# turswiming/UnSAMFlow

Measured on AMD Instinct MI355X. Metric: image-pairs/sec PWCLite fwd+bwd, KITTI 832x256 d=4, higher is better.
Workload: dtype f32; 1 GPU; PWCLite fwd(with_bk)+unFlowLoss+bwd+Adam, KITTI 832x256, d=4; global_batch=8, per_gpu_batch=8, max_displacement=4, parallelism=dp1

## Files before the change

### unsamflow_amd/_lib.py

```python
from __future__ import annotations

import ctypes
import os
import threading
from pathlib import Path

import torch

_LIB_PATH = Path(os.environ.get("USF_LIB", Path(__file__).resolve().parent / "lib" / "libunsamflow_hip.so"))
ABI_VERSION = 8
PAD_ZEROS = 0
PAD_BORDER = 1

_c_float_p = ctypes.c_void_p
_SIGNATURES = {
    "usf_abi_version": ([], ctypes.c_int),
    "usf_last_error_string": ([], ctypes.c_char_p),
    "usf_build_id": ([], ctypes.c_char_p),
    "usf_corr_fwd_f32": (
        [_c_float_p, _c_float_p, _c_float_p] + [ctypes.c_int] * 5 + [ctypes.c_void_p],
        ctypes.c_int,
    ),
    "usf_corr_bwd_f32": (
        [_c_float_p] * 5 + [ctypes.c_int] * 5 + [ctypes.c_void_p],
# ... 153 lines not shown
        [_c_float_p] * 3 + [ctypes.c_longlong] + [_c_float_p] * 8 + [ctypes.c_int] * 3 + [ctypes.c_void_p],
        ctypes.c_int,
    ),
    "usf_ar_loss_partials": ([ctypes.c_int] * 3, ctypes.c_int),
    "usf_ar_loss_fwd_f32": (
        [_c_float_p] + _ar_strided + [_c_float_p] * 3 + [ctypes.c_int] * 3 + [ctypes.c_float] * 2 + [ctypes.c_void_p],
        ctypes.c_int,
    ),
    "usf_ar_loss_bwd_f32": (
        [_c_float_p] + _ar_strided + [_c_float_p] * 3 + [ctypes.c_int] * 3 + [ctypes.c_float] * 2 + [ctypes.c_void_p],
        ctypes.c_int,
    ),
}

SEGPOOL_API_VERSION = 1
SEGPOOL_MAX_K = 1024
DEVERR_SEGPOOL_BAD_ID = 4
SEGPOOL_SYMBOLS = {
    "usf_segpool_api_version": ([], ctypes.c_int),
    "usf_segpool_state_words": ([ctypes.c_int] * 3, ctypes.c_longlong),
    "usf_segpool_fwd_f32": (
        [_c_float_p] * 3 + [ctypes.c_void_p] + [ctypes.c_int] * 5 + [ctypes.c_void_p],
        ctypes.c_int,
    ),
    "usf_segpool_bwd_f32": (
        [_c_float_p] * 2 + [ctypes.c_void_p] + [_c_float_p] * 2 + [ctypes.c_int] * 5 + [ctypes.c_void_p],
        ctypes.c_int,
    ),
}

HG_API_VERSION = 1
HG_MAX_K = 1024
HG_SLOTS = 6
HG_RECORD_WORDS = 16
HG_DEFAULT_HYP = 256
HG_STATUS = ("accepted", "too few reliable", "low reliable share", "low inlier share", "degenerate", "empty slot")
DEVERR_HG_BAD_ID = 8
_hg_flow = [_c_float_p, ctypes.c_longlong, _c_float_p]
HG_SYMBOLS = {
    "usf_hg_api_version": ([], ctypes.c_int),
    "usf_hg_workspace_bytes": ([ctypes.c_int] * 5, ctypes.c_longlong),
    "usf_hg_fit_f32": (
        _hg_flow + [_c_float_p, ctypes.c_int, ctypes.c_float, ctypes.c_int, ctypes.c_ulonglong, ctypes.c_void_p,
                    ctypes.c_void_p, ctypes.c_longlong] + [ctypes.c_int] * 3 + [ctypes.c_void_p],
        ctypes.c_int,
    ),
    "usf_hg_loss_partials": ([ctypes.c_int] * 3, ctypes.c_int),
    "usf_hg_loss_fwd_f32": (
        _hg_flow + [ctypes.c_void_p, ctypes.c_void_p, _c_float_p] + [ctypes.c_int] * 3 + [ctypes.c_void_p],
        ctypes.c_int,
    ),
    "usf_hg_loss_bwd_f32": (
        _hg_flow + [ctypes.c_void_p, _c_float_p, _c_float_p] + [ctypes.c_int] * 3 + [ctypes.c_void_p],
        ctypes.c_int,
    ),
}

_lock = threading.Lock()
_lib = None
_load_error: str | None = None


def library_path() -> Path:
    return _LIB_PATH


def load() -> ctypes.CDLL:
    global _lib, _load_error
    if _lib is not None:
        return _lib
    with _lock:
        if _lib is not None:
            return _lib
        if not _LIB_PATH.exists():
            _load_error = (
                f"libunsamflow_hip.so not found at {_LIB_PATH}; build it with "
                "`python -m unsamflow_amd.build` (hipcc, gfx950)"
            )
            raise RuntimeError(_load_error)
        lib = ctypes.CDLL(str(_LIB_PATH), mode=ctypes.RTLD_LOCAL)
        for name, (argtypes, restype) in {**_SIGNATURES, **CENSUS_SYMBOLS, **AR_SYMBOLS, **SEGPOOL_SYMBOLS,
                                          **HG_SYMBOLS}.items():
            fn = getattr(lib, name)
            fn.argtypes = argtypes
            fn.restype = restype
        v = lib.usf_abi_version()
        if v != ABI_VERSION:
            raise RuntimeError(f"libunsamflow_hip.so ABI version {v} != expected {ABI_VERSION}")
        v = lib.usf_census_api_version()
        if v != CENSUS_API_VERSION:
            raise RuntimeError(f"libunsamflow_hip.so census API version {v} != expected {CENSUS_API_VERSION}")
        v = lib.usf_ar_api_version()
        if v != AR_API_VERSION:
            raise RuntimeError(f"libunsamflow_hip.so AR API version {v} != expected {AR_API_VERSION}")
        v = lib.usf_segpool_api_version()
        if v != SEGPOOL_API_VERSION:
            raise RuntimeError(f"libunsamflow_hip.so segpool API version {v} != expected {SEGPOOL_API_VERSION}")
        v = lib.usf_hg_api_version()
        if v != HG_API_VERSION:
            raise RuntimeError(f"libunsamflow_hip.so hg API version {v} != expected {HG_API_VERSION}")
        _lib = lib
        return lib


def build_id() -> str:
    return load().usf_build_id().decode()


def is_available() -> bool:
    try:
        load()
        return True
    except (RuntimeError, OSError):
        return False


def check(rc: int, what: str) -> None:
    if rc != 0:
        msg = load().usf_last_error_string()
        msg = msg.decode() if msg else ""
        raise RuntimeError(f"{what} failed (rc={rc}): {msg}")


def stream_handle(device: torch.device) -> int:
    return torch.cuda.current_stream(device).cuda_stream
```

### unsamflow_amd/build.py

```python
from __future__ import annotations

import argparse
import hashlib
import os
import subprocess
import sys
from pathlib import Path

PKG_DIR = Path(__file__).resolve().parent
CSRC = PKG_DIR / "csrc"
LIB_DIR = PKG_DIR / "lib"
LIB_PATH = LIB_DIR / "libunsamflow_hip.so"
INCLUDE_DIR = PKG_DIR.parent / "include"

ARCH = os.environ.get("USF_OFFLOAD_ARCH", "gfx950")
HIPCC = os.environ.get("HIPCC", "/opt/rocm/bin/hipcc")

SOURCES = ["corr.hip", "warp.hip", "occ.hip", "photo.hip", "census.hip", "ar.hip", "segpool.hip", "hg.hip", "upsample.hip", "convex.hip", "stream.hip", "capi.cpp"]
HEADERS = ["usf_common.h", "warp_tap.h", "interp_tap.h", "strip.h", "wave.h", "scatter_rows.h", "seg_key.h"]
PUBLIC_HEADERS = ["unsamflow_hip.h", "unsamflow_hip_census.h", "unsamflow_hip_ar.h", "unsamflow_hip_segpool.h",
                  "unsamflow_hip_hg.h"]

COMMON_FLAGS = [
    "-O3",
    "-std=c++17",
    "-fno-slp-vectorize",
    "-fPIC",
    f"--offload-arch={ARCH}",
    "-Wall",
    "-Wno-unused-function",
    f"-I{INCLUDE_DIR}",
]


def build_id() -> str:
    h = hashlib.sha256()
    for f in [CSRC / s for s in SOURCES] + [CSRC / s for s in HEADERS] + [INCLUDE_DIR / s for s in PUBLIC_HEADERS]:
        h.update(f.name.encode())
        h.update(f.read_bytes())
    h.update(" ".join(COMMON_FLAGS).encode())
    return h.hexdigest()[:16]


def _stale(target: Path, deps: list[Path]) -> bool:
    if not target.exists():
        return True
    t = target.stat().st_mtime
    return any(d.stat().st_mtime > t for d in deps)


def build_library(force: bool = False, verbose: bool = False) -> Path:
    LIB_DIR.mkdir(exist_ok=True)
    obj_dir = LIB_DIR / "obj"
    obj_dir.mkdir(exist_ok=True)
    headers = [CSRC / h for h in HEADERS] + [INCLUDE_DIR / h for h in PUBLIC_HEADERS]
    bid = build_id()
    stamp = obj_dir / "build_id.txt"
    id_changed = not stamp.exists() or stamp.read_text().strip() != bid
    objs = []
    for src in SOURCES:
        s = CSRC / src
        o = obj_dir / (s.stem + ".o")
        objs.append(o)
        if force or _stale(o, [s] + headers) or (src == "capi.cpp" and id_changed):
            lang = ["-x", "hip"] if src.endswith(".hip") else []
            extra = [f'-DUSF_BUILD_ID="{bid}"'] if src == "capi.cpp" else []
            cmd = [HIPCC, *COMMON_FLAGS, *extra, *lang, "-c", str(s), "-o", str(o)]
            _run(cmd, verbose)
    stamp.write_text(bid + "\n")
    if force or _stale(LIB_PATH, objs):
        tmp = LIB_PATH.with_suffix(".so.tmp")
        cmd = [HIPCC, f"--offload-arch={ARCH}", "-shared", "-fPIC", *map(str, objs), "-o", str(tmp)]
        _run(cmd, verbose)
        os.replace(tmp, LIB_PATH)
# ... 26 lines not shown
```

### unsamflow_amd/csrc/capi.cpp

```cpp
#include <hip/hip_runtime.h>

#include <climits>
#include <cstdint>
#include <cstdarg>
#include <cstdio>
#include <cstdlib>

#include "../../include/unsamflow_hip.h"
#include "../../include/unsamflow_hip_ar.h"
#include "../../include/unsamflow_hip_census.h"
#include "../../include/unsamflow_hip_hg.h"
#include "../../include/unsamflow_hip_segpool.h"
#include "usf_common.h"

namespace usf {

static thread_local char g_err[512] = "";

void set_error(const char* fmt, ...) {
  va_list ap;
  va_start(ap, fmt);
  vsnprintf(g_err, sizeof(g_err), fmt, ap);
  va_end(ap);
}

void clear_error() { g_err[0] = '\0'; }

static bool check_dims(const char* fn, int B, int C, int H, int W) {
  if (B <= 0 || C <= 0 || H <= 0 || W <= 0) {
    set_error("%s: non-positive shape B=%d C=%d H=%d W=%d", fn, B, C, H, W);
    return false;
  }
  const long long per_sample = (long long)C * H * W;
  const long long max_elems = 0x7FFFFFF0LL / 4 - 1;
  if (per_sample > max_elems || (long long)H * W * 81 > max_elems) {
    set_error("%s: per-sample tensor too large (C*H*W=%lld)", fn, per_sample);
    return false;
  }
  return true;
}

static bool sync_check() {
  static const bool on = [] {
    const char* v = getenv("USF_SYNC_CHECK");
    return v && v[0] == '1';
  }();
  return on;
}

static bool capturing(hipStream_t s) {
  hipStreamCaptureStatus st = hipStreamCaptureStatusNone;
  return hipStreamIsCapturing(s, &st) == hipSuccess && st != hipStreamCaptureStatusNone;
}

static bool sync_check_on(hipStream_t s) { return sync_check() && !capturing(s); }

static int pre_check(const char* fn, hipStream_t s) {
  if (!sync_check_on(s)) return 0;
  const hipError_t e = hipStreamSynchronize(s);
  if (e != hipSuccess) {
    fprintf(stderr, "[usf] %s: stream already faulted BEFORE this launch: %s\n", fn, hipGetErrorString(e));
    set_error("%s: stream faulted before launch: %s (%d)", fn, hipGetErrorString(e), (int)e);
    return (int)e;
// ... 1086 lines not shown
    }
  if (const int pe = pre_check(fn, (hipStream_t)stream)) return pe;
  return finish(fn, convex_pyr_fwd_launch(nlevel, flow, mask, out, H, W, B, factor, mask_scale, (hipStream_t)stream),
                (hipStream_t)stream);
}

int usf_convex_upsample_pyramid_bwd_f32(int nlevel, const float* const* flow, const float* const* mask,
                                        const float* const* grad_out, float* const* grad_flow,
                                        float* const* grad_mask, float* scratch, long long scratch_floats,
                                        const int* H, const int* W, int B, int factor, float mask_scale,
                                        void* stream) {
  clear_error();
  const char* fn = "usf_convex_upsample_pyramid_bwd_f32";
  if (!check_convex_pyr(fn, nlevel, H, W, B, factor)) return USF_EINVAL;
  if (!flow || !mask || !grad_out) {
    set_error("%s: null input pointer array", fn);
    return USF_EINVAL;
  }
  for (int l = 0; l < nlevel; ++l)
    if (!flow[l] || !mask[l] || !grad_out[l] || (grad_flow && !grad_flow[l]) || (grad_mask && !grad_mask[l])) {
      set_error("%s: level %d: null pointer", fn, l);
      return USF_EINVAL;
    }
  if (grad_flow && (!scratch || scratch_floats < usf_convex_upsample_pyramid_bwd_scratch(nlevel, H, W, B))) {
    set_error("%s: grad_flow needs scratch of usf_convex_upsample_pyramid_bwd_scratch floats", fn);
    return USF_EINVAL;
  }
  if (!grad_flow && !grad_mask) return 0;
  if (const int pe = pre_check(fn, (hipStream_t)stream)) return pe;
  return finish(fn,
                convex_pyr_bwd_launch(nlevel, flow, mask, grad_out, grad_flow, grad_mask, scratch, H, W, B, factor,
                                      mask_scale, (hipStream_t)stream),
                (hipStream_t)stream);
}

int usf_area_pyramid_f32(const float* x, float* out1, float* out2, float* out3, int B, int C, int H,
                         int W, void* stream) {
  clear_error();
  const char* fn = "usf_area_pyramid_f32";
  if (!check_dims(fn, B, C, H, W)) return USF_EINVAL;
  if (H % 8 != 0 || W % 8 != 0) {
    set_error("%s: H=%d and W=%d must be multiples of 8", fn, H, W);
    return USF_EINVAL;
  }
  if (!x || !out1 || !out2 || !out3) {
    set_error("%s: null pointer", fn);
    return USF_EINVAL;
  }
  if (const int pe = pre_check(fn, (hipStream_t)stream)) return pe;
  return finish(fn, area_pyramid_launch(x, out1, out2, out3, (long long)B * C, H, W, (hipStream_t)stream),
                (hipStream_t)stream);
}

int usf_stream_copy_f32(const float* src, float* dst, long long n, void* stream) {
  clear_error();
  if (!src || !dst || n <= 0 || n % 4 != 0 || (reinterpret_cast<uintptr_t>(src) & 15) ||
      (reinterpret_cast<uintptr_t>(dst) & 15)) {
    set_error("usf_stream_copy_f32: need 16-byte aligned pointers and n %% 4 == 0 (n=%lld)", n);
    return USF_EINVAL;
  }
  if (const int pe = pre_check("usf_stream_copy_f32", (hipStream_t)stream)) return pe;
  return finish("usf_stream_copy_f32", stream_copy_launch(src, dst, n, (hipStream_t)stream), (hipStream_t)stream);
}

int usf_device_errors(void* stream, int clear) {
  clear_error();
  const int v = device_errors((hipStream_t)stream, clear != 0);
  if (v < 0) set_error("usf_device_errors: stream sync or flag read failed");
  return v;
}

int usf_set_variant(int op, int index) {
  clear_error();
  if (op < 0 || op > 3 || index < -1 || index >= variant_count(op)) {
    set_error("usf_set_variant: bad op %d / index %d", op, index);
    return USF_EINVAL;
  }
  set_variant_override(op, index);
  return variant_count(op);
}

}
```

### unsamflow_amd/csrc/usf_common.h

```cpp
#pragma once
#include <hip/hip_runtime.h>
#include <cstddef>
#include <cstdint>

#include "unsamflow_hip.h"

namespace usf {

int device_errors(hipStream_t s, bool clear, int mask = ~0);
template <class Sym>
int read_clear_flags(const Sym& word, bool clear, int mask = ~0) {
  int v = 0;
  if (hipMemcpyFromSymbol(&v, word, sizeof(int)) != hipSuccess) return -1;
  if (clear && (v & mask) != 0) {
    const int z = v & ~mask;
    if (hipMemcpyToSymbol(word, &z, sizeof(int)) != hipSuccess) return -1;
  }
  return v & mask;
}

void set_error(const char* fmt, ...);
void clear_error();

__host__ __device__ constexpr int round_up(int n, int m) { return ((n + m - 1) / m) * m; }
// ... 85 lines not shown
                                 int W, int pad_mode, float w_l1, float w_ssim, hipStream_t s);
hipError_t photo_pyr_fwd_launch(int nscale, const float* const* im1, const float* const* im2,
                                const float* const* mask1, const float* const* mask2, const float* const* flow,
                                const long long* fbs, const int* H, const int* W, float* partials, float* out,
                                float* const* basis, int B, int C, int pad_mode, float w_l1, float w_ssim,
                                hipStream_t s);
hipError_t photo_pyr_bwd_launch(int nscale, const float* const* basis, const float* coef, const float* gloss,
                                float* const* gflow, const int* H, const int* W, int B, int ndir, hipStream_t s);

int census_partials(int B, int H, int W);
hipError_t census_fwd_launch(const float* src, const float* tgt, const float* mask, const float* flow,
                             long long flow_bstride, float* partials, float* out, float* basis, int B, int H,
                             int W, int pad_mode, float w_ternary, hipStream_t s);
hipError_t census_pair_fwd_launch(const float* im1, const float* im2, const float* mask1, const float* mask2,
                                  const float* flow, long long flow_bstride, float* partials, float* out,
                                  float* basis, int B, int H, int W, int pad_mode, float w_ternary, hipStream_t s);
hipError_t census_pyr_fwd_launch(int nscale, const float* const* im1, const float* const* im2,
                                 const float* const* mask1, const float* const* mask2, const float* const* flow,
                                 const long long* fbs, const int* H, const int* W, float* partials, float* out,
                                 float* const* basis, int B, int pad_mode, float w_ternary, hipStream_t s);
hipError_t census_pyr_bwd_launch(int nscale, const float* const* basis, const float* coef, const float* gloss,
                                 float* const* gflow, const int* H, const int* W, int B, int ndir, hipStream_t s);

hipError_t ar_transform_launch(const float* img1, const float* img2, const float* flow, long long flow_bstride,
                               const float* mask, const float* theta, const float* noise1, const float* noise2,
                               float* img1_t, float* img2_t, float* flow_t, float* mask_t, int B, int H, int W,
                               hipStream_t s);
int ar_loss_partials(int B, int H, int W);
hipError_t ar_loss_fwd_launch(const float* pred, const float* target, long long tbs, long long tcs, long long trs,
                              const float* noc, long long nbs, long long nrs, const float* denom, float* partials,
                              float* out, int B, int H, int W, float eps, float q, hipStream_t s);
hipError_t ar_loss_bwd_launch(const float* pred, const float* target, long long tbs, long long tcs, long long trs,
                              const float* noc, long long nbs, long long nrs, const float* coef, const float* gloss,
                              float* gpred, int B, int H, int W, float eps, float q, hipStream_t s);

int segpool_device_errors(bool clear);
long long segpool_state_words(int B, int C, int K);
hipError_t segpool_fwd_launch(const float* proj, const float* seg, float* spread, unsigned* state, int B, int C,
                              int H, int W, int K, hipStream_t s);
hipError_t segpool_bwd_launch(const float* proj, const float* seg, const unsigned* state, const float* gs, float* gp,
                              int B, int C, int H, int W, int K, hipStream_t s);

int hg_device_errors(bool clear);
long long hg_workspace_bytes(int B, int H, int W, int K, int n_hyp);
hipError_t hg_fit_launch(const float* flow, long long fbs, const float* seg, const float* occ, int K, float thr,
                         int n_hyp, unsigned long long seed, int* records, void* workspace, int B, int H, int W,
                         hipStream_t s);
int hg_loss_partials(int B, int H, int W);
hipError_t hg_loss_fwd_launch(const float* flow, long long fbs, const float* seg, const int* records, double* partials,
                              float* out, int B, int H, int W, hipStream_t s);
hipError_t hg_loss_bwd_launch(const float* flow, long long fbs, const float* seg, const int* records,
                              const float* gloss, float* gflow, int B, int H, int W, hipStream_t s);

hipError_t upsample_fwd_launch(const float* x, float* out, int B, int C, int H, int W, int k,
                               hipStream_t s);
hipError_t upsample_bwd_launch(const float* gout, float* gx, int B, int C, int H, int W, int k,
                               hipStream_t s, const float* gout2 = nullptr);
int convex_pyramid_max_levels();
hipError_t convex_pyr_fwd_launch(int n, const float* const* flow, const float* const* mask, float* const* out,
                                 const int* H, const int* W, int B, int factor, float mask_scale, hipStream_t s);
hipError_t convex_pyr_bwd_launch(int n, const float* const* flow, const float* const* mask,
                                 const float* const* gout, float* const* gflow, float* const* gmask, float* scratch,
                                 const int* H, const int* W, int B, int factor, float mask_scale, hipStream_t s);
bool convex_factor_ok(int factor);
long long convex_bwd_scratch(int B, int H, int W);
hipError_t convex_fwd_launch(const float* flow, const float* mask, float* out, int B, int H, int W,
                             int factor, float mask_scale, hipStream_t s);
hipError_t convex_bwd_launch(const float* flow, const float* mask, const float* gout, float* gflow,
                             float* gmask, float* scratch, int B, int H, int W, int factor,
                             float mask_scale, hipStream_t s);
hipError_t stream_copy_launch(const float* src, float* dst, long long n, hipStream_t s);
hipError_t area_pyramid_launch(const float* x, float* o1, float* o2, float* o3, long long planes,
                               int H, int W, hipStream_t s);

}
```

### unsamflow_amd/kernel_timer.py

```python
from __future__ import annotations

import collections
import contextlib
import ctypes
import os

import torch

_active: "KernelTimer | None" = None
_roctx = None


def site_name(op: str, key) -> str:
    return "usf:" + op + ":" + "x".join(str(k) for k in key[:4]) + "".join(f":{k}" for k in key[4:])


def _roctx_lib():
    global _roctx
    if _roctx is None:
        _roctx = False
        if os.environ.get("USF_ROCTX") == "1":
            for name in ("librocprofiler-sdk-roctx.so.1", "librocprofiler-sdk-roctx.so", "libroctx64.so"):
                try:
                    lib = ctypes.CDLL(name)
# ... 57 lines not shown
        for a in agg.values():
            a["mean_us"] = a["total_us"] / a["n"]
        return agg


@contextlib.contextmanager
def timed(op: str, key, device, nbytes: int, flops: int = 0):
    rx = _roctx_lib()
    if rx:
        rx.roctxRangePushA(site_name(op, key).encode())
    try:
        kt = _active
        if kt is None or (kt.only is not None and (op, tuple(key)) not in kt.only):
            yield
            return
        if not kt.time_in_step:
            yield
            kt.records.append((op, key, None, None, nbytes, flops))
            return
        s = torch.cuda.Event(enable_timing=True)
        e = torch.cuda.Event(enable_timing=True)
        stream = torch.cuda.current_stream(device)
        s.record(stream)
        yield
        e.record(stream)
        kt.records.append((op, key, s, e, nbytes, flops))
    finally:
        if rx:
            rx.roctxRangePop()


def site_launcher(op: str, key, device, seed: int = 0):
    from . import ops

    g = torch.Generator(device=device).manual_seed(seed)
    if op == "corr_bwd_leaky":
        B, C, H, W = key[:4]
        x1 = torch.randn(B, C, H, W, device=device, generator=g)
        x2 = torch.randn(B, C, H, W, device=device, generator=g)
        cat = torch.randn(B, 81 + C + 2, H, W, device=device, generator=g)
        act = torch.nn.functional.leaky_relu(torch.randn(B, 81 + C + 2, H, W, device=device, generator=g), 0.1)
        mask = ops.corr_act_mask(B, H, W, 4, device, C=C)
        if mask is not None:
            ops.corr_forward_ex(x1, x2, 4, act[:, :81], 0.1, act_mask=mask)
        return lambda: ops.corr_backward_ex(x1, x2, cat[:, :81], 4, key[4], key[5], act_out=act[:, :81],
                                            act_mask=mask)
    if op == "corr_fwd_leaky":
        B, C, H, W = key[:4]
        x1 = torch.randn(B, C, H, W, device=device, generator=g)
        x2 = torch.randn(B, C, H, W, device=device, generator=g)
        cat = torch.empty(B, 81 + C + 2, H, W, device=device)
        mask = ops.corr_act_mask(B, H, W, 4, device, C=C)
        return lambda: ops.corr_forward_ex(x1, x2, 4, cat[:, :81], 0.1, act_mask=mask)
    if op in ("corr_fwd", "corr_bwd"):
        B, C, H, W = key[:4]
        x1 = torch.randn(B, C, H, W, device=device, generator=g)
        x2 = torch.randn(B, C, H, W, device=device, generator=g)
        if op == "corr_fwd":
            return lambda: ops.corr_forward(x1, x2, 4)
        need1, need2 = key[4], key[5]
        go = torch.randn(B, 81, H, W, device=device, generator=g)
        return lambda: ops.corr_backward(x1, x2, go, 4, need1, need2)
    if op in ("upsample", "upsample_bwd"):
        B, C, H, W, k = key[:5]
        if op == "upsample":
            f = torch.randn(B, C, H, W, device=device, generator=g)
            return lambda: ops.flow_upsample(f, k)
        go = torch.randn(B, C, H * k, W * k, device=device, generator=g)
        return lambda: ops.flow_upsample_backward(go, k)
    if op in ("convex_pyr", "convex_pyr_bwd"):
        B, f = key[0], key[-1]
        hw = [(key[i], key[i + 1]) for i in range(1, len(key) - 1, 2)]
        flows = [torch.randn(B, 2, h, w, device=device, generator=g) for h, w in hw]
        masks = [torch.randn(B, 9 * f * f, h, w, device=device, generator=g) for h, w in hw]
        if op == "convex_pyr":
            return lambda: ops.convex_upsample_pyramid(flows, masks, f)
        gos = [torch.randn(B, 2, f * h, f * w, device=device, generator=g) for h, w in hw]
        return lambda: ops.convex_upsample_pyramid_backward(flows, masks, gos, f)
    if op in ("convex_up", "convex_up_bwd"):
        B, H, W, f = key
        flow = torch.randn(B, 2, H, W, device=device, generator=g)
        mask = torch.randn(B, 9 * f * f, H, W, device=device, generator=g)
        if op == "convex_up":
            return lambda: ops.convex_upsample(flow, mask, f)
        go = torch.randn(B, 2, f * H, f * W, device=device, generator=g)
        return lambda: ops.convex_upsample_backward(flow, mask, go, f)
    if op == "area_pyramid":
        img = torch.rand(*key, device=device, generator=g)
        return lambda: ops.area_pyramid(img)
    if op == "photo_bwd":
        B, ndir, H, W = key
        basis = torch.randn(B, 4 * ndir, H, W, device=device, generator=g)
        coef = torch.rand(3 * ndir, device=device, generator=g)
        gl = torch.ones(ndir, device=device)
        return lambda: ops.photo_loss_backward(basis, coef, gl)
    if op == "census_bwd":
        B, ndir, H, W = key
        basis = torch.randn(B, 2 * ndir, H, W, device=device, generator=g)
        coef = torch.rand(2 * ndir, device=device, generator=g)
        gl = torch.ones(ndir, device=device)
        return lambda: ops.census_loss_backward(basis, coef, gl)
    if op in ("photo_pyr", "photo_pyr_grad", "photo_pyr_bwd", "census_pyr", "census_pyr_grad", "census_pyr_bwd"):
        B, C = key[:2]
        hw = [(key[i], key[i + 1]) for i in range(2, len(key) - (not op.endswith("_bwd")), 2)]
        if op == "census_pyr_bwd":
            bases = [torch.randn(B, 4, h, w, device=device, generator=g) for h, w in hw]
# ... 128 lines not shown
```

### unsamflow_amd/ops.py

```python
from __future__ import annotations

import ctypes
import weakref

import torch

from collections import OrderedDict, namedtuple

from . import _lib
from . import kernel_timer as _kt

PAD_MODES = {"zeros": _lib.PAD_ZEROS, "border": _lib.PAD_BORDER}


def _ptr(t: torch.Tensor | None) -> int | None:
    return None if t is None else t.data_ptr()


def _require_device_f32(name: str, t: torch.Tensor) -> None:
    if not isinstance(t, torch.Tensor):
        raise TypeError(f"{name} must be a torch.Tensor, got {type(t).__name__}")
    if t.device.type != "cuda":
        raise RuntimeError(
            f"unsamflow_amd: {name} is on {t.device}; the HIP kernels need tensors on a ROCm "
# ... 1000 lines not shown
    _args = (n, ptrs(fl), ptrs(mk), ptrs(outs), Hs, Ws, B, f_, float(mask_scale), _lib.stream_handle(dev),)
    with torch.cuda.device(dev), _kt.timed("convex_pyr", key, dev, nbytes):
        rc = lib.usf_convex_upsample_pyramid_f32(*_args)
    _lib.check(rc, "usf_convex_upsample_pyramid_f32")
    return outs


def convex_upsample_pyramid_backward(flows, masks, grad_outs, factor: int = 4, mask_scale: float = 0.25,
                                     need_flow: bool = True, need_mask: bool = True):
    import ctypes

    n = len(flows)
    fl = [f.contiguous() for f in flows]
    mk = [m.contiguous() for m in masks]
    go = [g.contiguous() for g in grad_outs]
    B, f_ = fl[0].shape[0], int(factor)
    if not (need_flow or need_mask):
        return None, None
    dev = fl[0].device
    gfs = [torch.empty((B, 2) + tuple(f.shape[2:]), device=dev, dtype=torch.float32) for f in fl] if need_flow else None
    gms = [torch.empty_like(m) for m in mk] if need_mask else None
    Hs, Ws = _level_sizes(fl)
    lib = _lib.load()
    nscr = int(lib.usf_convex_upsample_pyramid_bwd_scratch(n, Hs, Ws, B)) if need_flow else 0
    scratch = torch.empty(max(nscr, 1), device=dev, dtype=torch.float32)
    ptrs = lambda ts: _host_array(ctypes.c_void_p, [t.data_ptr() for t in ts])
    key = (B,) + tuple(v for f in fl for v in f.shape[2:]) + (f_,)
    ff = f_ * f_
    nbytes = sum(4 * B * f.shape[2] * f.shape[3] * (2 + 9 * ff + 2 * ff + (2 if need_flow else 0)
                                                    + (9 * ff if need_mask else 0)) for f in fl)
    _args = (n, ptrs(fl), ptrs(mk), ptrs(go), ptrs(gfs) if need_flow else None, ptrs(gms) if need_mask else None,
             scratch.data_ptr(), nscr, Hs, Ws, B, f_, float(mask_scale), _lib.stream_handle(dev),)
    with torch.cuda.device(dev), _kt.timed("convex_pyr_bwd", key, dev, nbytes):
        rc = lib.usf_convex_upsample_pyramid_bwd_f32(*_args)
    _lib.check(rc, "usf_convex_upsample_pyramid_bwd_f32")
    return gfs, gms


def area_pyramid(x: torch.Tensor):
    _require_device_f32("x", x)
    B, C, H, W = _nchw("x", x)
    if H % 8 or W % 8:
        raise ValueError(f"area_pyramid needs H, W multiples of 8, got {H}x{W}")
    xc = x.contiguous()
    outs = [torch.empty((B, C, H >> s, W >> s), device=x.device, dtype=torch.float32) for s in (1, 2, 3)]
    lib = _lib.load()
    nbytes = 4 * B * C * H * W * (1 + 1 / 4 + 1 / 16 + 1 / 64)
    _args = (xc.data_ptr(), outs[0].data_ptr(), outs[1].data_ptr(), outs[2].data_ptr(), B, C, H, W,
             _lib.stream_handle(x.device),)
    with torch.cuda.device(x.device), _kt.timed("area_pyramid", (B, C, H, W), x.device, int(nbytes)):
        rc = lib.usf_area_pyramid_f32(*_args)
    _lib.check(rc, "usf_area_pyramid_f32")
    return outs
```

### unsamflow_amd/pwclite.py

```python
from __future__ import annotations

from typing import Callable

import torch
import torch.nn as nn
import torch.nn.functional as F


def conv_block(cin: int, cout: int, k: int = 3, stride: int = 1, dilation: int = 1, relu: bool = True) -> nn.Sequential:
    layers = [nn.Conv2d(cin, cout, k, stride=stride, dilation=dilation, padding=((k - 1) * dilation) // 2, bias=True)]
    if relu:
        layers.append(nn.LeakyReLU(0.1, inplace=True))
    return nn.Sequential(*layers)


def full_segs_to_adj_maps(full_segs: torch.Tensor, win_size: int = 9, pad_mode: str = "replicate") -> torch.Tensor:
    r = (win_size - 1) // 2
    b, _, h, w = full_segs.shape
    nb = F.unfold(F.pad(full_segs, (r, r, r, r), mode=pad_mode), [win_size, win_size])
    return (full_segs == nb.reshape(b, win_size * win_size, h, w)).float()


class FeatureExtractor(nn.Module):
    def __init__(self, num_chs, input_adj_map: bool = False):
        super().__init__()
        self.num_chs = num_chs
        self.adj_map_net = None
        if input_adj_map:
            self.adj_map_net = nn.Sequential(
                conv_block(81, 32, k=1), conv_block(32, 32, stride=2), conv_block(32, 32),
                conv_block(32, 32, stride=2), conv_block(32, 32),
            )
        self.convs = nn.ModuleList()
        for lvl in range(len(num_chs) - 1):
            cin = num_chs[lvl] + (32 if input_adj_map and lvl == 2 else 0)
            cout = num_chs[lvl + 1]
            self.convs.append(nn.Sequential(conv_block(cin, cout, stride=2), conv_block(cout, cout)))

    def forward(self, x, adj_map=None):
        adj = self.adj_map_net(adj_map) if self.adj_map_net is not None else None
        pyramid = [x]
        for lvl, block in enumerate(self.convs):
            if adj is not None and lvl == 2:
                x = torch.cat((x, adj), dim=1)
            x = block(x)
            pyramid.append(x)
        return pyramid[::-1]


class FlowEstimatorDense(nn.Module):
    def __init__(self, ch_in: int):
        super().__init__()
        widths = [128, 128, 96, 64, 32]
        acc = ch_in
        for i, w in enumerate(widths, 1):
            setattr(self, f"conv{i}", conv_block(acc, w))
            acc += w
        self.feat_dim = acc
        self.conv_last = conv_block(acc, 2, relu=False)

    def forward(self, x):
        for i in range(1, 6):
            x = torch.cat([getattr(self, f"conv{i}")(x), x], dim=1)
        return x, self.conv_last(x)


# ... 15 lines not shown
        c = self.conv3(torch.cat([a, b], 1))
        d = self.conv4(torch.cat([b, c], 1))
        e = self.conv5(torch.cat([c, d], 1))
        return e, self.predict_flow(torch.cat([d, e], 1))


class ContextNetwork(nn.Module):
    def __init__(self, ch_in: int):
        super().__init__()
        self.convs = nn.Sequential(*[conv_block(ci, co, 3, 1, dil) for ci, co, dil in
                                     ((ch_in, 128, 1), (128, 128, 2), (128, 128, 4), (128, 96, 8))])
        self.flow_head = nn.Sequential(conv_block(96, 64, 3, 1, 16), conv_block(64, 32, 3, 1, 1),
                                       conv_block(32, 2, relu=False))

    def forward(self, x):
        feat = self.convs(x)
        return self.flow_head(feat), feat


class UpFlowNetwork(nn.Module):

    def __init__(self, ch_in: int = 96, scale_factor: int = 4):
        super().__init__()
        self.scale = scale_factor
        self.fused = False
        self.convs = nn.Sequential(conv_block(ch_in, 128, 3, 1, 1), conv_block(128, scale_factor ** 2 * 9, 3, 1, 1))

    def upsample_flow(self, flow, mask):
        N, _, H, W = flow.shape
        s = self.scale
        weights = torch.softmax(mask.view(N, 1, 9, s, s, H, W), dim=2)
        patches = F.unfold(s * flow, [3, 3], padding=1).view(N, 2, 9, 1, 1, H, W)
        up = torch.sum(weights * patches, dim=2)
        return up.permute(0, 1, 4, 2, 5, 3).reshape(N, 2, s * H, s * W)

    def mask(self, feat):
        return self.convs(feat)

    def forward(self, flow, feat):
        if self.fused and flow.is_cuda:
            from .upsample import convex_upsample

            return convex_upsample(flow, self.convs(feat), self.scale, 0.25)
        return self.upsample_flow(flow, 0.25 * self.convs(feat))


def _default_corr():
    from .correlation import Correlation

    return Correlation(pad_size=4, kernel_size=1, max_displacement=4, stride1=1, stride2=1, corr_multiply=1)


FUSED_UP_WARP = True
FUSED_SEG_POOL = True
SHARED_MASK_FEATURE = True


def _default_warp():
    from .warp_utils import flow_warp

    return flow_warp


class PWCLite(nn.Module):
    def __init__(self, cfg, corr_module: nn.Module | None = None, warp_fn: Callable | None = None):
        super().__init__()
        for key in ("input_adj_map", "input_boundary", "add_mask_corr"):
            if key not in cfg:
                cfg[key] = False
        self.cfg = cfg
        self.search_range = 4
        self.num_chs = [3, 16, 32, 64, 96, 128, 192]
        if cfg.input_boundary:
            self.num_chs[0] += 2
        self.output_level = 4
        self.batch_directions = True
        self.num_levels = 7
        self.leakyRELU = nn.LeakyReLU(0.1, inplace=True)
        self.warp = warp_fn if warp_fn is not None else _default_warp()

        self.feature_pyramid_extractor = FeatureExtractor(self.num_chs, input_adj_map=cfg.input_adj_map)
        self.corr = corr_module if corr_module is not None else _default_corr()
        self.fused_corr_cat = corr_module is None
        self.dim_corr = (2 * self.search_range + 1) ** 2
        self.num_ch_in = 32 + (2 if cfg.add_mask_corr else 1) * self.dim_corr + 2
        self.flow_estimators = (FlowEstimatorReduce if cfg.reduce_dense else FlowEstimatorDense)(self.num_ch_in)
        self.context_networks = ContextNetwork(self.flow_estimators.feat_dim + 2)
        self.output_flow_upsampler = UpFlowNetwork(ch_in=96, scale_factor=4) if cfg.learned_upsampler else None
        if self.output_flow_upsampler is not None:
            self.output_flow_upsampler.fused = self.fused_corr_cat
        level_chs = self.num_chs[::-1][:5]
        self.conv_1x1 = nn.ModuleList([conv_block(c, 32, k=1) for c in level_chs])
        if cfg.add_mask_corr:
            self.conv_1x1_mask = nn.ModuleList([conv_block(c, 32, k=1) for c in level_chs])
            if cfg.aggregation_type == "residual":
                self.mask_aggregation = conv_block(32, 32, k=1)
            elif cfg.aggregation_type == "concat":
                self.mask_aggregation = conv_block(64, 32, k=1)

    def num_parameters(self) -> int:
        return sum(p.numel() for p in self.parameters() if p.requires_grad)

    def _own_ops_on_device(self, x) -> bool:
        return self.fused_corr_cat and x.is_cuda

    def _segment_count(self, x, *full_segs):
        if not (self.cfg.add_mask_corr and FUSED_SEG_POOL and self._own_ops_on_device(x)):
            return None
        if "num_segments" in self.cfg:
            return int(self.cfg.num_segments)
        top = full_segs[0].max()
        for s in full_segs[1:]:
            top = torch.maximum(top, s.max())
        return int(top) + 1

    def _mask_feature(self, x, full_seg, level, num_segments=None):
        proj = self.conv_1x1_mask[level](x)
        seg = F.interpolate(full_seg, x.shape[-2:], mode="nearest")
        if FUSED_SEG_POOL and self._own_ops_on_device(x):
            from .segpool import segment_max_spread

            spread = segment_max_spread(proj, seg, num_segments)
        else:
            onehot = F.one_hot(seg.long())
            pooled = torch.amax(onehot * proj[..., None], dim=(2, 3))
            spread = (onehot * pooled[:, :, None, None, :]).sum(dim=-1)
        if self.cfg.aggregation_type == "residual":
            return proj + self.mask_aggregation(spread)
        if self.cfg.aggregation_type == "concat":
            return self.mask_aggregation(torch.cat((proj, spread), dim=1))
        raise NotImplementedError(self.cfg.aggregation_type)

    def _upsample(self, flow, k):
        if self.fused_corr_cat and flow.is_cuda:
            from .upsample import upsample_flow

            return upsample_flow(flow, k)
        return F.interpolate(flow * k, scale_factor=k, mode="bilinear", align_corners=True)

    def _fused_up_warp(self, flow):
        from .warp_utils import flow_warp

        return FUSED_UP_WARP and self.fused_corr_cat and flow.is_cuda and self.warp is flow_warp

    def decoder(self, x1_pyramid, x2_pyramid, full_seg1=None, full_seg2=None, num_segments=None,
                swapped_half=None):
        flows, deferred = [], []
        B, _, h0, w0 = x1_pyramid[0].size()
        flow = torch.zeros(B, 2, h0, w0, dtype=x1_pyramid[0].dtype, device=x1_pyramid[0].device).float()
        for level, (x1, x2) in enumerate(zip(x1_pyramid, x2_pyramid)):
            if level > 0 and self._fused_up_warp(flow):
# ... 84 lines not shown
```

Baseline: 202.6 image-pairs/s.

## Fuse conv bias-add and LeakyReLU into a custom in-place HIP epilogue

Every conv_block now runs the convolution without bias, then a custom HIP kernel adds the bias and applies LeakyReLU in place. The backward pass uses one kernel that masks the gradient by the sign of the output and reduces the bias gradient per channel, with a split-and-finish scheme. The aim is to replace the separate bias add, activation and bias-reduction passes that MIOpen/PyTorch would run with one fused read-modify-write. The risks are that bias-less conv kernels may be selected differently and that the custom kernels must beat vendor-fused conv+bias paths.

```diff
diff --git a/include/unsamflow_hip_convepi.h b/include/unsamflow_hip_convepi.h
--- /dev/null
+++ b/include/unsamflow_hip_convepi.h
@@ -0,0 +1,30 @@
+#ifndef UNSAMFLOW_HIP_CONVEPI_H
+#define UNSAMFLOW_HIP_CONVEPI_H
+
+#include "unsamflow_hip.h"
+
+#ifdef __cplusplus
+extern "C" {
+#endif
+
+#define USF_CONVEPI_API_VERSION 1
+
+#define USF_CONVEPI_TILE_SLOTS 1024
+#define USF_CONVEPI_CHAIN 64
+#define USF_CONVEPI_TARGET_WGS 16384
+
+int usf_convepi_api_version(void);
+
+int usf_convepi_fwd_f32(float* y, const float* bias, int B, int C, int H, int W, float slope, void* stream);
+
+long long usf_convepi_bwd_workspace(int B, int C, int H, int W);
+
+int usf_convepi_bwd_f32(const float* grad_out, long long gout_bstride, const float* y, float* grad_in,
+                        float* grad_bias, float* workspace, long long workspace_floats, int B, int C, int H, int W,
+                        float slope, void* stream);
+
+#ifdef __cplusplus
+}
+#endif
+
+#endif
diff --git a/unsamflow_amd/_lib.py b/unsamflow_amd/_lib.py
--- a/unsamflow_amd/_lib.py
+++ b/unsamflow_amd/_lib.py
@@ -229,6 +229,21 @@
     ),
     "usf_hg_loss_bwd_f32": (
         _hg_flow + [ctypes.c_void_p, _c_float_p, _c_float_p] + [ctypes.c_int] * 3 + [ctypes.c_void_p],
+        ctypes.c_int,
+    ),
+}
+
+CONVEPI_API_VERSION = 1
+CONVEPI_TILE_SLOTS = 1024
+CONVEPI_CHAIN = 64
+CONVEPI_TARGET_WGS = 16384
+CONVEPI_SYMBOLS = {
+    "usf_convepi_api_version": ([], ctypes.c_int),
+    "usf_convepi_fwd_f32": ([_c_float_p] * 2 + [ctypes.c_int] * 4 + [ctypes.c_float, ctypes.c_void_p], ctypes.c_int),
+    "usf_convepi_bwd_workspace": ([ctypes.c_int] * 4, ctypes.c_longlong),
+    "usf_convepi_bwd_f32": (
+        [_c_float_p, ctypes.c_longlong] + [_c_float_p] * 4 + [ctypes.c_longlong] + [ctypes.c_int] * 4
+        + [ctypes.c_float, ctypes.c_void_p],
         ctypes.c_int,
     ),
 }
@@ -257,7 +272,7 @@
             raise RuntimeError(_load_error)
         lib = ctypes.CDLL(str(_LIB_PATH), mode=ctypes.RTLD_LOCAL)
         for name, (argtypes, restype) in {**_SIGNATURES, **CENSUS_SYMBOLS, **AR_SYMBOLS, **SEGPOOL_SYMBOLS,
-                                          **HG_SYMBOLS}.items():
+                                          **HG_SYMBOLS, **CONVEPI_SYMBOLS}.items():
             fn = getattr(lib, name)
             fn.argtypes = argtypes
             fn.restype = restype
@@ -276,6 +291,9 @@
         v = lib.usf_hg_api_version()
         if v != HG_API_VERSION:
             raise RuntimeError(f"libunsamflow_hip.so hg API version {v} != expected {HG_API_VERSION}")
+        v = lib.usf_convepi_api_version()
+        if v != CONVEPI_API_VERSION:
+            raise RuntimeError(f"libunsamflow_hip.so convepi API version {v} != expected {CONVEPI_API_VERSION}")
         _lib = lib
         return lib
 
diff --git a/unsamflow_amd/build.py b/unsamflow_amd/build.py
--- a/unsamflow_amd/build.py
+++ b/unsamflow_amd/build.py
@@ -16,10 +16,10 @@
 ARCH = os.environ.get("USF_OFFLOAD_ARCH", "gfx950")
 HIPCC = os.environ.get("HIPCC", "/opt/rocm/bin/hipcc")
 
-SOURCES = ["corr.hip", "warp.hip", "occ.hip", "photo.hip", "census.hip", "ar.hip", "segpool.hip", "hg.hip", "upsample.hip", "convex.hip", "stream.hip", "capi.cpp"]
+SOURCES = ["corr.hip", "warp.hip", "occ.hip", "photo.hip", "census.hip", "ar.hip", "segpool.hip", "hg.hip", "upsample.hip", "convex.hip", "convepi.hip", "stream.hip", "capi.cpp"]
 HEADERS = ["usf_common.h", "warp_tap.h", "interp_tap.h", "strip.h", "wave.h", "scatter_rows.h", "seg_key.h"]
 PUBLIC_HEADERS = ["unsamflow_hip.h", "unsamflow_hip_census.h", "unsamflow_hip_ar.h", "unsamflow_hip_segpool.h",
-                  "unsamflow_hip_hg.h"]
+                  "unsamflow_hip_hg.h", "unsamflow_hip_convepi.h"]
 
 COMMON_FLAGS = [
     "-O3",
diff --git a/unsamflow_amd/conv_epilogue.py b/unsamflow_amd/conv_epilogue.py
--- /dev/null
+++ b/unsamflow_amd/conv_epilogue.py
@@ -0,0 +1,32 @@
+from __future__ import annotations
+
+import torch
+from torch.autograd import Function
+from torch.autograd.function import once_differentiable
+
+from . import ops
+
+
+class ConvEpilogueFunction(Function):
+    @staticmethod
+    def forward(ctx, raw, bias, slope):
+        ops.conv_epilogue_forward(raw, bias, slope)
+        ctx.mark_dirty(raw)
+        ctx.slope = float(slope)
+        if ctx.slope != 1.0:
+            ctx.save_for_backward(raw)
+        return raw
+
+    @staticmethod
+    @once_differentiable
+    def backward(ctx, grad_out):
+        y = ctx.saved_tensors[0] if ctx.slope != 1.0 else None
+        need_in, need_bias = ctx.needs_input_grad[:2]
+        if not need_in and not need_bias:
+            return None, None, None
+        gin, gbias = ops.conv_epilogue_backward(grad_out, y, ctx.slope, need_bias=need_bias)
+        return (gin if need_in else None), gbias, None
+
+
+def bias_act_(raw: torch.Tensor, bias: torch.Tensor, slope: float = 1.0) -> torch.Tensor:
+    return ConvEpilogueFunction.apply(raw, bias, slope)
diff --git a/unsamflow_amd/csrc/capi.cpp b/unsamflow_amd/csrc/capi.cpp
--- a/unsamflow_amd/csrc/capi.cpp
+++ b/unsamflow_amd/csrc/capi.cpp
@@ -9,6 +9,7 @@
 #include "../../include/unsamflow_hip.h"
 #include "../../include/unsamflow_hip_ar.h"
 #include "../../include/unsamflow_hip_census.h"
+#include "../../include/unsamflow_hip_convepi.h"
 #include "../../include/unsamflow_hip_hg.h"
 #include "../../include/unsamflow_hip_segpool.h"
 #include "usf_common.h"
@@ -1201,6 +1202,75 @@
                 (hipStream_t)stream);
 }
 
+int usf_convepi_api_version(void) { return USF_CONVEPI_API_VERSION; }
+
+static bool check_convepi(const char* fn, int B, int C, int H, int W, float slope) {
+  if (!check_dims(fn, B, C, H, W)) return false;
+  if (!(slope > 0.f)) {
+    set_error("%s: slope=%g (must be > 0)", fn, (double)slope);
+    return false;
+  }
+  return true;
+}
+
+int usf_convepi_fwd_f32(float* y, const float* bias, int B, int C, int H, int W, float slope, void* stream) {
+  clear_error();
+  const char* fn = "usf_convepi_fwd_f32";
+  if (!check_convepi(fn, B, C, H, W, slope)) return USF_EINVAL;
+  if (!y || !bias) {
+    set_error("%s: null pointer", fn);
+    return USF_EINVAL;
+  }
+  if ((uintptr_t)y % 16 != 0 || (uintptr_t)bias % 4 != 0) {
+    set_error("%s: y must be 16-byte and bias 4-byte aligned", fn);
+    return USF_EINVAL;
+  }
+  if (const int pe = pre_check(fn, (hipStream_t)stream)) return pe;
+  return finish(fn, convepi_fwd_launch(y, bias, B, C, H, W, slope, (hipStream_t)stream), (hipStream_t)stream);
+}
+
+long long usf_convepi_bwd_workspace(int B, int C, int H, int W) {
+  return (B > 0 && C > 0 && H > 0 && W > 0) ? convepi_bwd_workspace(B, C, H, W) : -1;
+}
+
+int usf_convepi_bwd_f32(const float* grad_out, long long gout_bstride, const float* y, float* grad_in,
+                        float* grad_bias, float* workspace, long long workspace_floats, int B, int C, int H, int W,
+                        float slope, void* stream) {
+  clear_error();
+  const char* fn = "usf_convepi_bwd_f32";
+  if (!check_convepi(fn, B, C, H, W, slope)) return USF_EINVAL;
+  const long long need = convepi_bwd_workspace(B, C, H, W);
+  if (need < 0) {
+    set_error("%s: shape B=%d C=%d H=%d W=%d too large for the bias-gradient split", fn, B, C, H, W);
+    return USF_EINVAL;
+  }
+  const bool act = slope != 1.f;
+  if (!grad_out || (uintptr_t)grad_out % 4 != 0 || gout_bstride < (long long)C * H * W) {
+    set_error("%s: grad_out null or misaligned, or gout_bstride=%lld < C*H*W", fn, gout_bstride);
+    return USF_EINVAL;
+  }
+  if (act ? (!y || !grad_in || (uintptr_t)y % 16 != 0 || (uintptr_t)grad_in % 16 != 0) : (y || grad_in)) {
+    set_error("%s: y and grad_in must be 16-byte aligned tensors with an activation, NULL without (slope=%g)", fn,
+              (double)slope);
+    return USF_EINVAL;
+  }
+  if (!grad_bias && !act) {
+    set_error("%s: nothing to compute (no activation and no grad_bias)", fn);
+    return USF_EINVAL;
+  }
+  if (grad_bias && ((uintptr_t)grad_bias % 4 != 0 ||
+                    (need > 0 && (!workspace || workspace_floats < need || (uintptr_t)workspace % 4 != 0)))) {
+    set_error("%s: grad_bias misaligned, or workspace of %lld floats null, misaligned or short (%lld given)", fn,
+              need, workspace_floats);
+    return USF_EINVAL;
+  }
+  if (const int pe = pre_check(fn, (hipStream_t)stream)) return pe;
+  return finish(fn,
+                convepi_bwd_launch(grad_out, gout_bstride, y, grad_in, grad_bias, workspace, B, C, H, W, slope,
+                                   (hipStream_t)stream),
+                (hipStream_t)stream);
+}
+
 int usf_stream_copy_f32(const float* src, float* dst, long long n, void* stream) {
   clear_error();
   if (!src || !dst || n <= 0 || n % 4 != 0 || (reinterpret_cast<uintptr_t>(src) & 15) ||
diff --git a/unsamflow_amd/csrc/convepi.hip b/unsamflow_amd/csrc/convepi.hip
--- /dev/null
+++ b/unsamflow_amd/csrc/convepi.hip
@@ -0,0 +1,215 @@
+#include "usf_common.h"
+#include "wave.h"
+
+#include "unsamflow_hip_convepi.h"
+
+namespace usf {
+namespace {
+
+using f4 = float __attribute__((ext_vector_type(4)));
+typedef f4 f4u __attribute__((aligned(4)));
+
+constexpr int THREADS = 256;
+constexpr int ROUNDS = 4;
+constexpr int TILE_SLOTS = USF_CONVEPI_TILE_SLOTS;
+static_assert(TILE_SLOTS == THREADS * ROUNDS, "a tile is four rounds of the workgroup");
+constexpr long long TARGET_WGS = USF_CONVEPI_TARGET_WGS;
+
+__device__ __forceinline__ float leaky(float v, float slope) { return v > 0.f ? v : v * slope; }
+
+__global__ __launch_bounds__(THREADS) void convepi_fwd_kernel(float* __restrict__ y, const float* __restrict__ bias,
+                                                             long long n, int C, int HW, float slope) {
+  const long long tile0 = (long long)blockIdx.x * (TILE_SLOTS * 4);
+  const long long p0 = tile0 / HW;
+  const int r0 = (int)(tile0 - p0 * HW);
+  const int c0 = (int)(p0 % C);
+  f4 v[ROUNDS];
+  int rr[ROUNDS], cc[ROUNDS];
+#pragma unroll
+  for (int k = 0; k < ROUNDS; ++k) {
+    const int off = 4 * (k * THREADS + (int)threadIdx.x);
+    const long long i = tile0 + off;
+    int r = r0 + off, c = c0;
+    if (HW >= TILE_SLOTS * 4) {
+      if (r >= HW) {
+        r -= HW;
+        c = c + 1 == C ? 0 : c + 1;
+      }
+    } else {
+      const int dp = r / HW;
+      r -= dp * HW;
+      c = (c + dp) % C;
+    }
+    rr[k] = r;
+    cc[k] = c;
+    if (i + 4 <= n) v[k] = *reinterpret_cast<const f4*>(y + i);
+  }
+#pragma unroll
+  for (int k = 0; k < ROUNDS; ++k) {
+    const long long i = tile0 + 4 * (k * THREADS + (int)threadIdx.x);
+    int r = rr[k], c = cc[k];
+    if (i + 4 <= n && r + 4 <= HW) {
+      const float b = bias[c];
+      f4 o;
+      o.x = leaky(v[k].x + b, slope);
+      o.y = leaky(v[k].y + b, slope);
+      o.z = leaky(v[k].z + b, slope);
+      o.w = leaky(v[k].w + b, slope);
+      *reinterpret_cast<f4*>(y + i) = o;
+    } else {
+      for (int e = 0; e < 4; ++e) {
+        if (i + e < n) y[i + e] = leaky(y[i + e] + bias[c], slope);
+        if (++r == HW) {
+          r = 0;
+          c = c + 1 == C ? 0 : c + 1;
+        }
+      }
+    }
+  }
+}
+
+template <bool ACT, bool RED>
+__global__ __launch_bounds__(THREADS) void convepi_bwd_kernel(const float* __restrict__ gout, long long gbs,
+                                                             const float* __restrict__ y, float* __restrict__ gin,
+                                                             float* __restrict__ sums, int B, int C, int HW, int nsm,
+                                                             int tiles, int tpp, int parts, float slope) {
+  const int c = blockIdx.x / parts, part = blockIdx.x - c * parts;
+  const int t_end = min(tiles, (part + 1) * tpp);
+  const unsigned L0 = (unsigned)part * tpp * TILE_SLOTS + threadIdx.x;
+  int b = (int)(L0 / (unsigned)nsm);
+  int j = (int)(L0 - (unsigned)b * nsm);
+  f4 acc[ROUNDS];
+#pragma unroll
+  for (int k = 0; k < ROUNDS; ++k) acc[k] = f4{0.f, 0.f, 0.f, 0.f};
+  for (int t = part * tpp; t < t_end; ++t) {
+    f4 g[ROUNDS], a[ROUNDS];
+    long long dense[ROUNDS], go[ROUNDS];
+    int e0s[ROUNDS];
+    bool full[ROUNDS], live[ROUNDS];
+#pragma unroll
+    for (int k = 0; k < ROUNDS; ++k) {
+      const long long start = ((long long)b * C + c) * HW;
+      const int e0 = 4 * j - (int)(start & 3);
+      live[k] = b < B && e0 < HW;
+      full[k] = live[k] && e0 >= 0 && e0 + 4 <= HW;
+      e0s[k] = e0;
+      dense[k] = start + e0;
+      go[k] = (long long)b * gbs + (long long)c * HW + e0;
+      j += THREADS;
+      if (nsm >= THREADS) {
+        if (j >= nsm) {
+          j -= nsm;
+          ++b;
+        }
+      } else {
+        const int db = j / nsm;
+        j -= db * nsm;
+        b += db;
+      }
+      if (full[k]) {
+        g[k] = *reinterpret_cast<const f4u*>(gout + go[k]);
+        if (ACT) a[k] = *reinterpret_cast<const f4*>(y + dense[k]);
+      }
+    }
+#pragma unroll
+    for (int k = 0; k < ROUNDS; ++k) {
+      if (full[k]) {
+        f4 o = g[k];
+        if (ACT) {
+          o.x = a[k].x > 0.f ? o.x : o.x * slope;
+          o.y = a[k].y > 0.f ? o.y : o.y * slope;
+          o.z = a[k].z > 0.f ? o.z : o.z * slope;
+          o.w = a[k].w > 0.f ? o.w : o.w * slope;
+          *reinterpret_cast<f4*>(gin + dense[k]) = o;
+        }
+        if (RED) acc[k] += o;
+      } else if (live[k]) {
+        float edge = 0.f;
+        for (int e = 0; e < 4; ++e) {
+          const int pe = e0s[k] + e;
+          if (pe < 0 || pe >= HW) continue;
+          float v = gout[go[k] + e];
+          if (ACT) {
+            v = y[dense[k] + e] > 0.f ? v : v * slope;
+            gin[dense[k] + e] = v;
+          }
+          edge += v;
+        }
+        if (RED) acc[k].x += edge;
+      }
+    }
+  }
+  if (!RED) return;
+  const f4 s4 = (acc[0] + acc[1]) + (acc[2] + acc[3]);
+  const float lane_sum = wave_sum((s4.x + s4.y) + (s4.z + s4.w));
+  __shared__ float wsum[THREADS / 64];
+  if ((threadIdx.x & 63) == 0) wsum[threadIdx.x >> 6] = lane_sum;
+  __syncthreads();
+  if (threadIdx.x == 0) sums[blockIdx.x] = (wsum[0] + wsum[1]) + (wsum[2] + wsum[3]);
+}
+
+__global__ __launch_bounds__(64) void convepi_finish_kernel(const float* __restrict__ partials,
+                                                           float* __restrict__ gbias, int parts) {
+  const float* p = partials + (long long)blockIdx.x * parts;
+  float s = 0.f;
+  for (int i = threadIdx.x; i < parts; i += 64) s += p[i];
+  s = wave_sum(s);
+  if (threadIdx.x == 0) gbias[blockIdx.x] = s;
+}
+
+struct Split {
+  int nsm, tiles, tpp, parts;
+};
+
+bool bwd_split(int B, int C, int H, int W, Split* sp) {
+  const long long HW = (long long)H * W;
+  const long long nsm = (HW + 3 + 3) / 4;
+  if ((long long)B * nsm > 0x7FF00000LL) return false;
+  const long long tiles = ((long long)B * nsm + TILE_SLOTS - 1) / TILE_SLOTS;
+  long long tpp = (tiles * C + TARGET_WGS - 1) / TARGET_WGS;
+  if (tpp > USF_CONVEPI_CHAIN) tpp = USF_CONVEPI_CHAIN;
+  if (tpp < 1) tpp = 1;
+  const long long parts = (tiles + tpp - 1) / tpp;
+  if (parts > 64 * USF_CONVEPI_CHAIN || parts * C > 0x7FFFFFFFLL) return false;
+  *sp = Split{(int)nsm, (int)tiles, (int)tpp, (int)parts};
+  return true;
+}
+
+}
+
+long long convepi_bwd_workspace(int B, int C, int H, int W) {
+  Split sp;
+  if (!bwd_split(B, C, H, W, &sp)) return -1;
+  return sp.parts > 1 ? (long long)C * sp.parts : 0;
+}
+
+hipError_t convepi_fwd_launch(float* y, const float* bias, int B, int C, int H, int W, float slope, hipStream_t s) {
+  const long long n = (long long)B * C * H * W;
+  const long long tiles = (n + TILE_SLOTS * 4 - 1) / (TILE_SLOTS * 4);
+  hipLaunchKernelGGL(convepi_fwd_kernel, dim3((unsigned)tiles), dim3(THREADS), 0, s, y, bias, n, C, H * W, slope);
+  return hipGetLastError();
+}
+
+hipError_t convepi_bwd_launch(const float* gout, long long gbs, const float* y, float* gin, float* gbias,
+                              float* workspace, int B, int C, int H, int W, float slope, hipStream_t s) {
+  Split sp;
+  if (!bwd_split(B, C, H, W, &sp)) return hipErrorInvalidValue;
+  const bool act = slope != 1.f, red = gbias != nullptr;
+  float* sums = sp.parts > 1 ? workspace : gbias;
+  const dim3 grid((unsigned)(C * sp.parts)), block(THREADS);
+#define USF_CONVEPI_BWD(ACT, RED)                                                                                  \
+  hipLaunchKernelGGL((convepi_bwd_kernel<ACT, RED>), grid, block, 0, s, gout, gbs, y, gin, sums, B, C, H * W, sp.nsm, \
+                     sp.tiles, sp.tpp, sp.parts, slope)
+  if (act && red) USF_CONVEPI_BWD(true, true);
+  else if (act) USF_CONVEPI_BWD(true, false);
+  else USF_CONVEPI_BWD(false, true);
+#undef USF_CONVEPI_BWD
+  hipError_t e = hipGetLastError();
+  if (e == hipSuccess && red && sp.parts > 1) {
+    hipLaunchKernelGGL(convepi_finish_kernel, dim3((unsigned)C), dim3(64), 0, s, workspace, gbias, sp.parts);
+    e = hipGetLastError();
+  }
+  return e;
+}
+
+}
diff --git a/unsamflow_amd/csrc/usf_common.h b/unsamflow_amd/csrc/usf_common.h
--- a/unsamflow_amd/csrc/usf_common.h
+++ b/unsamflow_amd/csrc/usf_common.h
@@ -161,6 +161,11 @@
 hipError_t hg_loss_bwd_launch(const float* flow, long long fbs, const float* seg, const int* records,
                               const float* gloss, float* gflow, int B, int H, int W, hipStream_t s);
 
+long long convepi_bwd_workspace(int B, int C, int H, int W);
+hipError_t convepi_fwd_launch(float* y, const float* bias, int B, int C, int H, int W, float slope, hipStream_t s);
+hipError_t convepi_bwd_launch(const float* gout, long long gbs, const float* y, float* gin, float* gbias,
+                              float* workspace, int B, int C, int H, int W, float slope, hipStream_t s);
+
 hipError_t upsample_fwd_launch(const float* x, float* out, int B, int C, int H, int W, int k,
                                hipStream_t s);
 hipError_t upsample_bwd_launch(const float* gout, float* gx, int B, int C, int H, int W, int k,
diff --git a/unsamflow_amd/kernel_timer.py b/unsamflow_amd/kernel_timer.py
--- a/unsamflow_amd/kernel_timer.py
+++ b/unsamflow_amd/kernel_timer.py
@@ -133,6 +133,15 @@
         cat = torch.empty(B, 81 + C + 2, H, W, device=device)
         mask = ops.corr_act_mask(B, H, W, 4, device, C=C)
         return lambda: ops.corr_forward_ex(x1, x2, 4, cat[:, :81], 0.1, act_mask=mask)
+    if op in ("conv_epi_fwd", "conv_epi_bwd"):
+        B, C, H, W, act = key[:5]
+        slope = 0.1 if act else 1.0
+        bias = torch.randn(C, device=device, generator=g)
+        y = torch.randn(B, C, H, W, device=device, generator=g)
+        if op == "conv_epi_fwd":
+            return lambda: ops.conv_epilogue_forward(y, bias, slope)
+        go = torch.randn(B, C, H, W, device=device, generator=g)
+        return lambda: ops.conv_epilogue_backward(go, y if act else None, slope)
     if op in ("corr_fwd", "corr_bwd"):
         B, C, H, W = key[:4]
         x1 = torch.randn(B, C, H, W, device=device, generator=g)
diff --git a/unsamflow_amd/ops.py b/unsamflow_amd/ops.py
--- a/unsamflow_amd/ops.py
+++ b/unsamflow_amd/ops.py
@@ -1076,3 +1076,78 @@
         rc = lib.usf_area_pyramid_f32(*_args)
     _lib.check(rc, "usf_area_pyramid_f32")
     return outs
+
+
+def _conv_epi_args(y, bias, slope):
+    _require_device_f32("y", y)
+    _require_device_f32("bias", bias)
+    B, C, H, W = _nchw("y", y)
+    if not y.is_contiguous():
+        raise ValueError(f"y must be dense NCHW (strides {y.stride()})")
+    if tuple(bias.shape) != (C,) or bias.device != y.device:
+        raise ValueError(f"bias must be [{C}] on {y.device}, got {tuple(bias.shape)} on {bias.device}")
+    slope = float(slope)
+    if not slope > 0.0:
+        raise ValueError(f"slope={slope} must be > 0 (1 = no activation)")
+    return B, C, H, W, slope
+
+
+def conv_epilogue_forward(raw: torch.Tensor, bias: torch.Tensor, slope: float = 1.0) -> torch.Tensor:
+    B, C, H, W, slope = _conv_epi_args(raw, bias, slope)
+    if raw.numel() == 0:
+        return raw
+    dev = raw.device
+    lib = _lib.load()
+    _args = (raw.data_ptr(), bias.contiguous().data_ptr(), B, C, H, W, slope, _lib.stream_handle(dev),)
+    with torch.cuda.device(dev), _kt.timed("conv_epi_fwd", (B, C, H, W, slope != 1.0), dev,
+                                           8 * B * C * H * W + 4 * C):
+        rc = lib.usf_convepi_fwd_f32(*_args)
+    _lib.check(rc, "usf_convepi_fwd_f32")
+    return raw
+
+
+def conv_epilogue_backward(grad_out: torch.Tensor, y: torch.Tensor | None, slope: float,
+                           need_bias: bool = True) -> tuple[torch.Tensor, torch.Tensor | None]:
+    _require_device_f32("grad_out", grad_out)
+    B, C, H, W = _nchw("grad_out", grad_out)
+    slope = float(slope)
+    if not slope > 0.0:
+        raise ValueError(f"slope={slope} must be > 0 (1 = no activation)")
+    act = slope != 1.0
+    dev = grad_out.device
+    if act:
+        if y is None:
+            raise ValueError("y (the forward's result) is needed with an activation")
+        _require_device_f32("y", y)
+        if tuple(y.shape) != (B, C, H, W) or y.device != dev or not y.is_contiguous():
+            raise ValueError(f"y must be a dense {(B, C, H, W)} tensor on {dev}")
+    elif y is not None:
+        raise ValueError("y must be None without an activation (slope == 1)")
+    if not act and not need_bias:
+        return grad_out, None
+    if grad_out.numel() == 0:
+        return (torch.empty_like(y) if act else grad_out), (grad_out.new_zeros(C) if need_bias else None)
+    try:
+        gbs = _plane_slice_stride("grad_out", grad_out, (B, C, H, W))
+        g = grad_out
+    except ValueError:
+        g = grad_out.contiguous()
+        gbs = C * H * W
+    lib = _lib.load()
+    gin = torch.empty((B, C, H, W), device=dev, dtype=torch.float32) if act else None
+    gbias = ws = None
+    nws = 0
+    if need_bias:
+        nws = int(lib.usf_convepi_bwd_workspace(B, C, H, W))
+        if nws < 0:
+            raise ValueError(f"conv_epilogue_backward: shape {(B, C, H, W)} is too large for the bias-gradient split")
+        gbias = torch.empty(C, device=dev, dtype=torch.float32)
+        if nws:
+            ws = torch.empty(nws, device=dev, dtype=torch.float32)
+    _args = (g.data_ptr(), gbs, _ptr(y), _ptr(gin), _ptr(gbias), _ptr(ws), nws, B, C, H, W, slope,
+             _lib.stream_handle(dev),)
+    with torch.cuda.device(dev), _kt.timed("conv_epi_bwd", (B, C, H, W, act), dev,
+                                           (12 if act else 4) * B * C * H * W + 4 * C):
+        rc = lib.usf_convepi_bwd_f32(*_args)
+    _lib.check(rc, "usf_convepi_bwd_f32")
+    return (gin if act else grad_out), gbias
diff --git a/unsamflow_amd/pwclite.py b/unsamflow_amd/pwclite.py
--- a/unsamflow_amd/pwclite.py
+++ b/unsamflow_amd/pwclite.py
@@ -5,13 +5,38 @@
 import torch
 import torch.nn as nn
 import torch.nn.functional as F
+
+
+def _channels_last(t: torch.Tensor) -> bool:
+    return t.dim() == 4 and not t.is_contiguous() and t.is_contiguous(memory_format=torch.channels_last)
+
+
+class ConvBlock(nn.Sequential):
+
+    fused = True
+
+    def forward(self, x):
+        conv = self[0]
+        slope = self[1].negative_slope if len(self) > 1 else 1.0
+        if not (FUSED_CONV_EPILOGUE and self.fused and x.is_cuda and x.dtype == torch.float32
+                and conv.weight.dtype == torch.float32 and conv.bias is not None and slope > 0
+                and not _channels_last(x) and not _channels_last(conv.weight)
+                and not torch.is_autocast_enabled()):
+            return super().forward(x)
+        from .conv_epilogue import bias_act_
+
+        raw = conv._conv_forward(x, conv.weight, None)
+        if not raw.is_contiguous():
+            raw = raw + conv.bias.view(1, -1, 1, 1)
+            return self[1](raw) if len(self) > 1 else raw
+        return bias_act_(raw, conv.bias, slope)
 
 
 def conv_block(cin: int, cout: int, k: int = 3, stride: int = 1, dilation: int = 1, relu: bool = True) -> nn.Sequential:
     layers = [nn.Conv2d(cin, cout, k, stride=stride, dilation=dilation, padding=((k - 1) * dilation) // 2, bias=True)]
     if relu:
         layers.append(nn.LeakyReLU(0.1, inplace=True))
-    return nn.Sequential(*layers)
+    return ConvBlock(*layers)
 
 
 def full_segs_to_adj_maps(full_segs: torch.Tensor, win_size: int = 9, pad_mode: str = "replicate") -> torch.Tensor:
@@ -133,6 +158,7 @@
 
 
 FUSED_UP_WARP = True
+FUSED_CONV_EPILOGUE = True
 FUSED_SEG_POOL = True
 SHARED_MASK_FEATURE = True
 
@@ -178,6 +204,10 @@
                 self.mask_aggregation = conv_block(32, 32, k=1)
             elif cfg.aggregation_type == "concat":
                 self.mask_aggregation = conv_block(64, 32, k=1)
+        if not self.fused_corr_cat:
+            for m in self.modules():
+                if isinstance(m, ConvBlock):
+                    m.fused = False
 
     def num_parameters(self) -> int:
         return sum(p.numel() for p in self.parameters() if p.requires_grad)
```

Result: faster. 215.4 image-pairs/s, median of 6 (+6.3%).
